# jeremy-rifkin/Markov-Huffman-Coding

Hardware: AMD Instinct MI355X
Metric: encode+decode GB/s on 16 GB byte stream, bit-exact round-trip (higher is better)
Workload: dtype u8

## Files before the change

markov-huffman-coding_amd/csrc/mh_api.cpp:

```cpp
#include "mh_api_internal.hpp"

namespace mhapi {

thread_local int g_last_hip = 0;
thread_local int g_encode_retries = 0;
std::atomic<uint64_t> g_encode_retries_total{0};
thread_local int g_last_index_path = 0;

class PinnedRing {
public:
    static constexpr size_t PIECE = size_t(16) << 20;
    static constexpr int SLOTS = 4;
    hipError_t upload(void *d_dst, const void *h_src, size_t n, hipStream_t st) {
        std::lock_guard<std::mutex> lock(mu_);
        hipError_t e = ensure();
        if (e != hipSuccess) return e;
        const unsigned char *src = static_cast<const unsigned char *>(h_src);
        unsigned char *dst = static_cast<unsigned char *>(d_dst);
        for (size_t off = 0; off < n; off += PIECE, ++seq_) {
            const size_t len = std::min(PIECE, n - off);
            const int s = int(seq_ % SLOTS);
            if ((e = hipEventSynchronize(ev_[s])) != hipSuccess) return e;
            parallel_copy(buf_[s], src + off, len);
            if ((e = hipMemcpyAsync(dst + off, buf_[s], len, hipMemcpyHostToDevice, st)) != hipSuccess) return e;
// ... 363 lines not shown
    p.direct = m->dec_direct ? 1u : 0u; p.H = uint32_t(m->dec_h);
    const int path = decode_path_choice();
    const bool tile_ok = d_fine && path != 2 && (m->type == 2 ? (m->o2_dec_ok && shift <= 10) : (m->tile_p && shift <= 12));
    const bool long_codes = m->type != 2 && nbits && n_symbols && double(nbits) > (double(m->tile_p) - 0.5) * double(n_symbols);
    if (tile_ok && (path == 1 || (n_symbols >= (uint64_t(8) << 20) && !long_codes))) {
        mhk::TileParams t{};
        t.payload = d_payload; t.payload_bytes = p.payload_bytes; t.nbits = nbits; t.d_nbits = p.d_nbits;
        t.out = d_out; t.n = n_symbols; t.index = p.index; t.nchunks = p.nchunks; t.chunk_shift = p.chunk_shift;
        t.fine = d_fine;
        t.prim = m->d_tprim; t.sec = m->d_tsec; t.P = uint32_t(m->tile_p); t.H = uint32_t(m->tile_h); t.nsec = m->tile_nsec;
        if (m->type == 2) {
            t.o2 = 1; t.nslots = m->o2_nslots; t.ctx2slot = m->d_ctx2slot;
            t.prim = reinterpret_cast<const uint16_t *>(m->d_tprim2); t.sec = reinterpret_cast<const uint16_t *>(m->d_tsec2);
            t.P = m->o2_p; t.H = m->o2_h; t.nsec = m->o2_nsec;
        }
        HIP_TRY(mhk::launch_decode_tile(t, p, d_ws, static_cast<hipStream_t>(stream)));
        HIP_TRY(mhk::launch_set_word(reinterpret_cast<uint32_t *>(static_cast<unsigned char *>(d_ws) + 40), mhk::DEC_PATH_TILE, static_cast<hipStream_t>(stream)));
        return MH_OK;
    }
    HIP_TRY(mhk::launch_decode(p, d_ws, static_cast<hipStream_t>(stream)));
    HIP_TRY(mhk::launch_set_word(reinterpret_cast<uint32_t *>(static_cast<unsigned char *>(d_ws) + 40), mhk::DEC_PATH_CHUNK, static_cast<hipStream_t>(stream)));
    return MH_OK;
}

int mh_dev_decode_fine(const mh_model *m, const uint8_t *d_payload, uint64_t nbits, const uint64_t *d_nbits, uint8_t *d_out,
                       uint64_t n_symbols, const uint64_t *d_index, uint32_t chunk_symbols, const uint32_t *d_fine,
                       void *d_ws, size_t ws_bytes, void *stream) {
    return dev_decode(m, d_payload, nbits, d_nbits, d_out, n_symbols, d_index, chunk_symbols, d_ws, ws_bytes, stream, d_fine);
}

int mh_dev_decode(const mh_model *m, const uint8_t *d_payload, uint64_t nbits, uint8_t *d_out, uint64_t n_symbols,
                  const uint64_t *d_index, uint32_t chunk_symbols, void *d_ws, size_t ws_bytes, void *stream) {
    return dev_decode(m, d_payload, nbits, nullptr, d_out, n_symbols, d_index, chunk_symbols, d_ws, ws_bytes, stream);
}

int mh_dev_decode_dn(const mh_model *m, const uint8_t *d_payload, const uint64_t *d_nbits, uint64_t nbits_hint, uint8_t *d_out,
// ... 118 lines not shown
```

markov-huffman-coding_amd/csrc/mh_api_model.cpp:

```cpp
#include "mh_api_internal.hpp"
#include "mh_limit.hpp"

namespace mhapi {

int upload_model(mh_model *m) {
    m->packed = m->host.pack();
    m->type = m->host.type;
    m->max_len = m->packed.max_len;
    m->dec_bits = m->packed.dec_bits; m->dec_h = m->packed.dec_h;
    m->dec_lds = m->packed.dec_lds; m->dec_direct = m->packed.dec_direct;
    m->nsec = uint32_t(m->packed.dec_sec.size());
    for (size_t i = 0; i < size_t(256) * 256; ++i) {
        const int l = m->packed.len8[i];
        if (l && (m->min_len == 0 || l < m->min_len)) m->min_len = l;
    }
    for (int c = 0; c < 256; ++c) {
        int live = 0;
        for (int sy = 0; sy < 256; ++sy) live += m->packed.len8[size_t(c) * 256 + sy] != 0;
        if (live < 2) continue;
        for (int sy = 0; sy < 256; ++sy) m->len_gcd = gcd_u32(m->len_gcd, m->packed.len8[size_t(c) * 256 + sy]);
    }
    if (!have_device()) return MH_OK;
    if (m->max_len > mh::MAX_CODE_BITS) return MH_OK;
    HIP_TRY(hipGetDevice(&m->device));
// ... 200 lines not shown
    for (int i = 0; i < 256; ++i) {
        const int c = order_idx[i];
        const uint32_t *mt = &meta[size_t(c) * mhk::TB_META_STRIDE];
        pa.sec_base_val[c] = uint32_t(nsec);
        nsec += m->dec_direct ? (size_t(mt[3]) << m->dec_h) : size_t(mt[4 + P]);
    }
    m->nsec = uint32_t(nsec);
    const size_t sec_bytes = ((nsec * 2 + 15) & ~size_t(15)) + 16;
    if (d_ws) {
        if (ws_bytes < L.fixed + sec_bytes) return fail(MH_ERR_CAPACITY);
        m->d_sec = reinterpret_cast<uint16_t *>(b + L.fixed);
    } else {
        HIP_TRY_M(hipMalloc(&m->d_sec_own, sec_bytes));
        m->d_sec = static_cast<uint16_t *>(m->d_sec_own);
    }
    HIP_TRY_M(hipMemsetAsync(m->d_sec, 0, sec_bytes, st));
    pa.node_left = m->d_node_left; pa.node_right = m->d_node_right; pa.node_sym = m->d_node_sym; pa.node_height = d_node_height;
    pa.ctx_meta = m->d_meta; pa.sec_base = m->d_sec_base;
    pa.P = uint32_t(P); pa.direct = m->dec_direct ? 1u : 0u; pa.H = uint32_t(m->dec_h); pa.hcap = 8u;
    pa.prim = m->d_prim; pa.sec = m->d_sec; pa.tree = m->d_tree;
    bool packed = false;
    if (const int tP = tile_p_choice()) {
        const int tH = std::min(std::max(m->max_len - tP, 1), 8);
        size_t ntab = size_t(256) << tP;
        mhk::TreePackArgs pt{};
        if (tP == 8) {
            ntab = 0;
            for (int c = 0; c < 256; ++c) { pt.sec_base_val[c] = uint32_t(ntab << tH); ntab += meta[size_t(c) * mhk::TB_META_STRIDE + 3]; }
        } else {
            for (int c = 0; c < 256; ++c) pt.sec_base_val[c] = uint32_t(size_t(c) << (tP + tH));
        }
        if (ntab <= 32767 || tP < 8) {
            const size_t pb = ((size_t(256) << tP) * 2 + 255) & ~size_t(255), sb = (ntab << tH) * 2 + 64;
            unsigned char *tb;
            if (d_ws) {
                const size_t at = (L.fixed + sec_bytes + 255) & ~size_t(255);
                if (ws_bytes < at + pb + sb) return fail(MH_ERR_CAPACITY);
                tb = b + at;
            } else {
                HIP_TRY_M(hipMalloc(&m->d_tile_own, pb + sb));
                tb = static_cast<unsigned char *>(m->d_tile_own);
            }
            m->d_tprim = reinterpret_cast<uint16_t *>(tb);
            m->d_tsec = reinterpret_cast<uint16_t *>(tb + pb);
            HIP_TRY_M(hipMemsetAsync(m->d_tsec, 0, sb, st));
            pt.node_left = m->d_node_left; pt.node_right = m->d_node_right; pt.node_sym = m->d_node_sym; pt.node_height = d_node_height;
            pt.ctx_meta = m->d_meta; pt.sec_base = nullptr; pt.sec_base_in = nullptr;
            pt.P = uint32_t(tP); pt.direct = 1u; pt.H = uint32_t(tH); pt.hcap = 8u;
            pt.prim = m->d_tprim; pt.sec = m->d_tsec; pt.tree = nullptr; pt.lsb = 1u;
            HIP_TRY_M(mhk::launch_tree_pack2(pa, pt, 256, st));
            packed = true;
            m->tile_p = tP; m->tile_h = tH; m->tile_nsec = uint32_t(ntab << tH);
        }
    }
    if (!packed) HIP_TRY_M(mhk::launch_tree_pack(pa, 256, st));
#undef HIP_TRY_M
    *out = m;
    return MH_OK;
}
}

namespace {
constexpr uint32_t O2_CTX = 65536;
constexpr uint32_t O2_HCAP = 4;
const unsigned char O2_MAGIC[4] = {'M', 'H', '2', 1};

bool is_o2_table(const uint8_t *b, size_t n) {
    if (n < 37 || b[0] != 0x80) return false;
    for (int i = 1; i < 33; ++i) if (b[i]) return false;
// ... 505 lines not shown
```

markov-huffman-coding_amd/csrc/mh_decode.hip:

```cpp
#include "mh_decode_dev.hpp"

namespace mhk {

template <typename LS>
__device__ __forceinline__ bool walk_long(const DecTables &t, LS &ls, uint32_t prev, uint32_t e2, uint32_t skip,
                                          uint32_t &sym) {
    ls.buf <<= skip; ls.cnt -= skip;
    uint32_t node = e2 & 0x1FFu;
    const uint32_t *tr = t.tree + prev * TREE_STRIDE;
    for (int guard = 0; guard < 256; ++guard) {
        ls.template refill<true>();
        uint32_t bit = uint32_t(ls.buf >> 63);
        ls.buf <<= 1; ls.cnt -= 1u;
        uint32_t pair = tr[node];
        uint32_t c = bit ? (pair >> 16) : (pair & 0xFFFFu);
        if (c & TREE_LEAF) { sym = c & 255u; ls.template refill<true>(); return true; }
        node = c;
    }
    sym = 0;
    return false;
}

#ifndef MH_DEC_LAG
#define MH_DEC_LAG 1
// ... 128 lines not shown
    }
    for (uint32_t i = nsym & ~3u; i < nsym; ++i) o[i] = uint8_t(q >> (8u * (i & 3u)));
    if (bad || ls[0].position() != uint32_t(end_bits)) atomicExch(status, MHK_STATUS_CORRUPT);
}

template <int K, int OUTB, int NT>
__device__ __forceinline__ void store_burst(const DecParams &p, uint64_t c0, const uint32_t (&Q)[K][OUTB][4], uint32_t b) {
#pragma unroll
    for (int k = 0; k < K; ++k) {
        uint4 *o16 = reinterpret_cast<uint4 *>(p.out + ((c0 + uint64_t(k) * NT) << p.chunk_shift)) + b * OUTB;
#pragma unroll
        for (int u = 0; u < OUTB; ++u) o16[u] = make_uint4(Q[k][u][0], Q[k][u][1], Q[k][u][2], Q[k][u][3]);
    }
}

struct DecCfg { bool sec_lds; int spr; int k, gw, outb, pc, hc; bool redo; int depth; };
__host__ __device__ constexpr DecCfg dec_cfg(int v) {
    return v == DV_LDS_WIDE       ? DecCfg{true, 4, 2, 16, 4, 8, 0, false, 2}
         : v == DV_LDS_SHORT      ? DecCfg{true, 4, 4, 8, 2, 8, 0, false, 2}
         : v == DV_LDS_TWO_LEVEL  ? DecCfg{true, 2, 4, 8, 2, 0, 0, false, 2}
         : v == DV_LDS_TWO_LEVEL_P8 ? DecCfg{true, 2, 4, 8, 2, 8, 0, false, 2}
         : v == DV_L2_DIRECT      ? DecCfg{false, 2, 4, 8, 4, 8, 0, false, 1}
         : v == DV_L2_DIRECT_H2   ? DecCfg{false, 2, 4, 8, 4, 8, 2, false, 1}
         : v == DV_L2_DIRECT_H3   ? DecCfg{false, 2, 4, 8, 4, 8, 3, false, 1}
         : v == DV_L2_DIRECT_H4   ? DecCfg{false, 2, 4, 8, 4, 8, 4, false, 1}
         : v == DV_L2_DIRECT_H8   ? DecCfg{false, 2, 4, 8, 4, 8, 8, false, 1}
         : v == DV_REDO_LDS       ? DecCfg{true, 2, 1, 8, 1, 0, 0, true, 2}
                                  : DecCfg{false, 2, 1, 8, 1, 0, 0, true, 2};
}
constexpr int DEC_NT = 512;
template <int V>
__global__ __launch_bounds__(DEC_NT) void decode_kernel(DecParams p) {
    constexpr DecCfg C = dec_cfg(V);
    constexpr bool SEC_LDS = C.sec_lds, DIRECT = !C.sec_lds, REDO = C.redo;
    constexpr int SPR = C.spr, K = C.k, GW = C.gw, OUTB = C.outb, PC = C.pc, HC = C.hc, NT = DEC_NT, DEPTH = C.depth;
    extern __shared__ __attribute__((aligned(16))) unsigned char smem[];
    if (REDO && p.redo[0] == 0) return;
    if (p.d_nbits) {
        p.nbits = *p.d_nbits;
        p.payload_bytes = (p.nbits + 7) >> 3;
    }
    uint32_t *sub_base = reinterpret_cast<uint32_t *>(smem);
    uint16_t *lut = reinterpret_cast<uint16_t *>(smem + 1024);
    const uint32_t nprim16 = (256u << p.P) / 8u;
    for (uint32_t i = threadIdx.x; i < nprim16; i += NT)
        reinterpret_cast<uint4 *>(lut)[i] = reinterpret_cast<const uint4 *>(p.prim)[i];
    uint16_t *lsec = lut + (256u << p.P);
    if (SEC_LDS) {
        const uint32_t nsec16 = (p.nsec + 7u) / 8u;
        for (uint32_t i = threadIdx.x; i < nsec16; i += NT)
            reinterpret_cast<uint4 *>(lsec)[i] = reinterpret_cast<const uint4 *>(p.sec)[i];
// ... 93 lines not shown
        } else {
            for (int k = 0; k < K; ++k) {
                const uint64_t c = c0 + uint64_t(k) * NT;
                if (c >= p.nchunks) break;
                const uint64_t first = c << p.chunk_shift;
                const uint32_t nsym = (p.n - first) >= S ? S : uint32_t(p.n - first);
                const uint64_t endb = (c + 1 < p.nchunks) ? (p.index[c + 1] & 0x00FFFFFFFFFFFFFFull) : p.nbits;
                decode_chunk_single<DIRECT>(lut, sub_base, tabs, p.payload, p.payload_bytes, p.nbits, p.index[c], endb, p.out + first, nsym, p.status);
            }
        }
    }
}


__global__ __launch_bounds__(256) void decode2_kernel(DecParams p) {
    if (p.d_nbits) { p.nbits = *p.d_nbits; p.payload_bytes = (p.nbits + 7) >> 3; }
    const BitSrc src{p.payload, p.payload_bytes >> 2, p.payload_bytes};
    const DecTables tabs{p.sec, p.tree, p.P, 0u, 0u};
    const uint32_t S = 1u << p.chunk_shift;
    const uint64_t nwork = p.redo_list ? uint64_t(p.redo[0]) : p.nchunks;
    for (uint64_t w = uint64_t(blockIdx.x) * blockDim.x + threadIdx.x; w < nwork; w += uint64_t(gridDim.x) * blockDim.x) {
        const uint64_t c = p.redo_list ? uint64_t(p.redo[1u + w]) : w;
        const uint64_t entry = p.index[c];
        uint64_t pos = entry & IDX2_POS;
        uint32_t ctx = uint32_t(entry >> 48);
        const uint64_t endpos = (c + 1 < p.nchunks) ? (p.index[c + 1] & IDX2_POS) : p.nbits;
        const uint64_t first = c << p.chunk_shift;
        const uint32_t nsym = (p.n - first) >= S ? S : uint32_t(p.n - first);
        if (pos >= p.nbits || endpos < pos || endpos > p.nbits) { atomicExch(p.status, MHK_STATUS_CORRUPT); continue; }
        GranuleCursor bc;
// ... 26 lines not shown
            for (int u = 0; u < 4; ++u) o16[u] = Q[u];
        }
        for (; i < nsym && !bad; ++i) {
            uint32_t used = 0;
            const uint32_t sym = decode_one(p.prim, p.sec_base, tabs, src, bc, ctx, used, bad);
            pos += used;
            ctx = ((ctx << 8) | sym) & 0xFFFFu;
            o[i] = uint8_t(sym);
        }
        if (bad || pos != endpos) atomicExch(p.status, MHK_STATUS_CORRUPT);
    }
}


hipError_t launch_decode_redo(DecParams p, hipStream_t st) {
    if (p.order == 2) {
        p.redo_list = 1;
        const uint64_t want2 = (p.nchunks + 255) / 256;
        const uint64_t cap2 = uint64_t(cu_count()) * 8;
        hipLaunchKernelGGL(decode2_kernel, dim3(unsigned(want2 > cap2 ? cap2 : (want2 < 1 ? 1 : want2))), dim3(256), 0, st, p);
        return hipGetLastError();
    }
    auto r_lds = decode_kernel<DV_REDO_LDS>;
    auto r_l2d = decode_kernel<DV_REDO_L2_DIRECT>;
    hipError_t e = once_per_device(&DeviceState::redo_ready, [&] {
        const void *all[] = {(const void *)r_lds, (const void *)r_l2d};
        for (const void *f : all) {
            hipError_t r = allow_lds(f, DEC_LDS_MAX);
            if (r != hipSuccess) return r;
        }
// ... 2 lines not shown
    if (e != hipSuccess) return e;
    if (!p.sec_lds && !p.direct) return hipErrorInvalidValue;
    if (!p.sec_lds && p.P != 8) return hipErrorInvalidValue;
    const size_t lds = 1024 + (size_t(256) << p.P) * 2 + (p.sec_lds ? ((size_t(p.nsec) * 2 + 15) & ~size_t(15)) : 0);
    if (lds > size_t(DEC_LDS_MAX)) return hipErrorInvalidValue;
    const uint64_t rwant = (p.nchunks + DEC_THREADS - 1) / DEC_THREADS;
    const int rgrid = int(rwant > uint64_t(cu_count()) ? uint64_t(cu_count()) : rwant);
    hipLaunchKernelGGL(p.sec_lds ? r_lds : r_l2d, dim3(rgrid < 1 ? 1 : rgrid), dim3(DEC_THREADS), lds, st, p);
    return hipGetLastError();
}

hipError_t launch_decode(DecParams p, void *d_ws, hipStream_t st) {
    p.status = reinterpret_cast<int *>(d_ws);
    p.redo = reinterpret_cast<uint32_t *>(static_cast<char *>(d_ws) + 64);
    hipError_t e = hipMemsetAsync(d_ws, 0, 64 + 16, st);
    if (e != hipSuccess || p.nchunks == 0) return e;
    if (p.order == 2) {
        const uint64_t want2 = (p.nchunks + 255) / 256;
        const uint64_t cap2 = uint64_t(cu_count()) * 8;
        hipLaunchKernelGGL(decode2_kernel, dim3(unsigned(want2 > cap2 ? cap2 : want2)), dim3(256), 0, st, p);
        return hipGetLastError();
    }
    if (!p.sec_lds && (p.P != 8 || !p.direct)) return hipErrorInvalidValue;
    size_t lds = 1024 + (size_t(256) << p.P) * 2 + (p.sec_lds ? ((size_t(p.nsec) * 2 + 15) & ~size_t(15)) : 0);
    if (lds > size_t(DEC_LDS_MAX)) return hipErrorInvalidValue;
    const bool short_codes = p.nsec == 0 && p.P == 8;
    const bool wide = p.sec_lds && short_codes && p.n > 0 && p.nbits * 10 > p.n * 8 * 6;
    int v;
    if (wide) v = DV_LDS_WIDE;
    else if (p.sec_lds) v = short_codes ? DV_LDS_SHORT : p.P == 8 ? DV_LDS_TWO_LEVEL_P8 : DV_LDS_TWO_LEVEL;
    else v = p.H == 2 ? DV_L2_DIRECT_H2 : p.H == 3 ? DV_L2_DIRECT_H3 : p.H == 4 ? DV_L2_DIRECT_H4 : p.H == 8 ? DV_L2_DIRECT_H8 : DV_L2_DIRECT;
    void (*const kern[DV_REDO_LDS])(DecParams) = {decode_kernel<DV_LDS_WIDE>, decode_kernel<DV_LDS_SHORT>, decode_kernel<DV_LDS_TWO_LEVEL>,
                                                  decode_kernel<DV_LDS_TWO_LEVEL_P8>, decode_kernel<DV_L2_DIRECT>, decode_kernel<DV_L2_DIRECT_H2>,
                                                  decode_kernel<DV_L2_DIRECT_H3>, decode_kernel<DV_L2_DIRECT_H4>, decode_kernel<DV_L2_DIRECT_H8>};
    static_assert(DV_LDS_WIDE == 0 && DV_L2_DIRECT_H8 == 8 && DV_REDO_LDS == 9, "the table above is indexed by DecVariant");
    e = once_per_device(&DeviceState::decode_ready, [&] {
        for (int i = 0; i < DV_REDO_LDS; ++i) {
            hipError_t r = allow_lds(reinterpret_cast<const void *>(kern[i]), DEC_LDS_MAX);
            if (r != hipSuccess) return r;
        }
        return hipSuccess;
    });
    if (e != hipSuccess) return e;
    const uint64_t per_block = uint64_t(DEC_NT) * uint64_t(dec_cfg(v).k);
    const uint64_t want = (p.nchunks + per_block - 1) / per_block;
    const int grid = int(want > uint64_t(cu_count()) ? uint64_t(cu_count()) : want);
    (void)launch_set_word(reinterpret_cast<uint32_t *>(static_cast<char *>(d_ws) + 44), uint32_t(v) + 1u, st);
    hipLaunchKernelGGL(kern[v], dim3(grid), dim3(DEC_NT), lds, st, p);
    e = hipGetLastError();
    if (e != hipSuccess) return e;
    return launch_decode_redo(p, st);
}


}
```

markov-huffman-coding_amd/csrc/mh_encode.hip:

```cpp
#include "mh_dev.hpp"

namespace mhk {


constexpr uint32_t O2H_MAP_OFF = 256, O2H_HOT_OFF = 256 + 64 * 64 * 2;
__device__ __forceinline__ void o2hot_lookup16(const unsigned char *img, const uint4 &x4, uint32_t ctx, uint32_t (&e)[16]) {
    const uint16_t *ctxmap = reinterpret_cast<const uint16_t *>(img + O2H_MAP_OFF);
    const uint16_t *hot = reinterpret_cast<const uint16_t *>(img + O2H_HOT_OFF);
    const uint32_t x[4] = {x4.x, x4.y, x4.z, x4.w};
    uint32_t id[18];
    id[0] = img[ctx >> 8];
    id[1] = img[ctx & 255u];
#pragma unroll
    for (int j = 0; j < 16; ++j) id[2 + j] = img[(x[j >> 2] >> (8 * (j & 3))) & 255u];
    uint32_t cs[16];
#pragma unroll
    for (int j = 0; j < 16; ++j) cs[j] = ctxmap[(id[j] << 6) | (id[j + 1] ^ id[j])];
#pragma unroll
    for (int j = 0; j < 16; ++j) e[j] = hot[(cs[j] << 6) | (id[j + 2] ^ id[j + 1])];
}

__device__ __forceinline__ void o2hot_lookup8(const unsigned char *img, uint32_t xa, uint32_t xb, uint32_t ctx, uint32_t (&e)[8]) {
    const uint16_t *ctxmap = reinterpret_cast<const uint16_t *>(img + O2H_MAP_OFF);
    const uint16_t *hot = reinterpret_cast<const uint16_t *>(img + O2H_HOT_OFF);
// ... 629 lines not shown
            } else if (cur != 0 && lane == 0) {
                stage[0] = 0;
            }
        }
    }
}

constexpr int R_IMG_WORDS = ((163840 - 131072 - 128) / 4) & ~7;
constexpr int R_HALF_WORDS = R_IMG_WORDS / 2;
constexpr uint32_t R_HALF_CAP_BITS = uint32_t(R_HALF_WORDS - 8) * 32u;
static_assert(R_IMG_WORDS >= E_WAVES * (E_STAGE_BITS / 32) + 16 && R_HALF_WORDS % 4 == 0, "image size");
constexpr int REGION_LDS_BYTES = 131072 + R_IMG_WORDS * 4 + 128;



__global__ __launch_bounds__(1024) void region_bits_kernel(const HistHeader *hdr, HistHeader expect, const uint32_t *slab,
                                                           const uint32_t *cross_all, const uint8_t *len8,
                                                           unsigned long long *region_bits, uint32_t *region_esc, int *status) {
    __shared__ unsigned long long part[16];
    __shared__ uint32_t any_esc;
    extern __shared__ __attribute__((aligned(16))) unsigned char lens[];
    for (uint32_t i = threadIdx.x; i < 65536u / 16u; i += 1024u) reinterpret_cast<uint4 *>(lens)[i] = reinterpret_cast<const uint4 *>(len8)[i];
    if (threadIdx.x == 0) any_esc = 0;
    __syncthreads();
    const uint32_t w = blockIdx.x, tid = threadIdx.x;
    if (hdr->magic != HIST_WS_MAGIC || hdr->n != expect.n || hdr->data != expect.data || hdr->region_vecs != expect.region_vecs ||
        hdr->grid != expect.grid || hdr->prev0 != expect.prev0 || hdr->cross_cap != expect.cross_cap) {
        if (tid == 0) { atomicExch(status, MHK_STATUS_CORRUPT); region_bits[w] = 0; region_esc[w] = 0; }
        return;
    }
    unsigned long long acc = 0;
    bool esc = false;
    const uint32_t *sl = slab + size_t(w) * 32768u;
    for (uint32_t i = tid; i < 32768u; i += 1024u) {
        const uint32_t v = sl[i];
        const uint32_t s0 = i, s1 = i | 0x8000u;
        const uint32_t l0 = lens[hist_slot_prev(s0) * 256u + (s0 >> 8)], l1 = lens[hist_slot_prev(s1) * 256u + (s1 >> 8)];
        acc += (unsigned long long)(v & 0xFFFFu) * l0;
        acc += (unsigned long long)(v >> 16) * l1;
        esc |= ((v & 0xFFFFu) && l0 > uint32_t(mh::ENC16_MAX_LEN)) || ((v >> 16) && l1 > uint32_t(mh::ENC16_MAX_LEN));
    }
    const uint32_t *cross = cross_all + size_t(w) * (expect.cross_cap + 1u);
    const uint32_t nc = cross[0];
    if (nc > expect.cross_cap && tid == 0) atomicExch(status, MHK_STATUS_CAPACITY);
    for (uint32_t i = tid; i < (nc < expect.cross_cap ? nc : expect.cross_cap); i += 1024u) {
        const uint32_t sl2 = cross[1u + i];
        const uint32_t l2 = lens[hist_slot_prev(sl2) * 256u + (sl2 >> 8)];
        acc += 16384ull * l2;
        esc |= l2 > uint32_t(mh::ENC16_MAX_LEN);
    }
    if (esc) atomicOr(&any_esc, 1u);
    for (int d = 32; d >= 1; d >>= 1) acc += __shfl_xor(acc, d);
    if ((tid & 63u) == 0) part[tid >> 6] = acc;
    __syncthreads();
    if (tid == 0) {
        unsigned long long t = 0;
        for (int i = 0; i < 16; ++i) t += part[i];
        region_bits[w] = t;
        region_esc[w] = any_esc;
    }
}

__global__ __launch_bounds__(SCAN_THREADS) void region_scan_kernel(const unsigned long long *region_bits, uint32_t nregion,
                                                                   unsigned long long *region_start, const unsigned long long *carry0,
                                                                   uint8_t *out, uint64_t cap, unsigned long long *nbits, int *status) {
    __shared__ uint64_t lds[SCAN_THREADS / 64];
    const uint64_t c0 = carry0 ? (*carry0 & 7ull) : 0;
    const uint32_t i = threadIdx.x;
    const uint64_t v = i < nregion ? region_bits[i] : 0;
    uint64_t total;
    const uint64_t ex = block_excl_scan(v, lds, total);
    const uint64_t s = c0 + ex;
    if (i < nregion) {
        region_start[i] = s;
        if (i > 0 && (s & 31u) && ((s >> 5) + 1) * 4 <= cap) reinterpret_cast<uint32_t *>(out)[s >> 5] = 0;
    }
    if (i == 0) {
        const uint64_t end = c0 + total;
        *nbits = end;
        if (end > cap * 8) atomicExch(status, MHK_STATUS_CAPACITY);
        const uint64_t endw = end >> 5;
        if ((end & 31u) && (endw + 1) * 4 <= cap) reinterpret_cast<uint32_t *>(out)[endw] = 0;
        else if (end & 31u) for (uint64_t b = endw * 4; b < cap; ++b) out[b] = 0;
        if ((c0 & 31u) && 4 <= cap) reinterpret_cast<uint32_t *>(out)[0] = 0;
    }
}

struct RegionParams {
    const unsigned long long *region_start;
    const unsigned long long *region_bits;
    const uint32_t *region_esc;
    uint64_t region_vecs;
    uint64_t nvec_up;
    uint64_t cap_words;
    int *status;
};
constexpr uint32_t R_IMG_CAP_BITS = E_WAVES * E_STAGE_BITS;

struct Roll1 {
// ... 538 lines not shown

hipError_t launch_encode_regions(const EncodeArgs &a, const void *d_hist_ws, size_t hist_ws_bytes, void *d_ws, hipStream_t st) {
    unsigned char *ws = static_cast<unsigned char *>(d_ws);
    int *status = reinterpret_cast<int *>(ws);
    hipError_t e = hipMemsetAsync(ws, 0, 64, st);
    if (e != hipSuccess) return e;
    if (a.n == 0) {
        hipLaunchKernelGGL(empty_payload_kernel, dim3(1), dim3(1), 0, st, a.start_bit, a.nbits, a.out, a.cap);
        return hipGetLastError();
    }
    const RegionGeom g = region_geom(a.n);
    if (!d_hist_ws || hist_ws_bytes < g.total || g.grid > 1024) return hipErrorInvalidValue;
    e = once_per_device(&DeviceState::region_ready, [] {
        hipError_t r = allow_lds(reinterpret_cast<const void *>(enc_region_kernel<false>), REGION_LDS_BYTES);
        if (r == hipSuccess) r = allow_lds(reinterpret_cast<const void *>(enc_region_kernel<false, true>), REGION_LDS_BYTES);
        if (r == hipSuccess) r = allow_lds(reinterpret_cast<const void *>(region_bits_kernel), 65536);
        return r != hipSuccess ? r : allow_lds(reinterpret_cast<const void *>(enc_region_kernel<true>), REGION_LDS_BYTES);
    });
    if (e != hipSuccess) return e;
    const unsigned char *hws = static_cast<const unsigned char *>(d_hist_ws);
    unsigned long long *region_bits = reinterpret_cast<unsigned long long *>(ws + 64);
    unsigned long long *region_start = region_bits + 1024;
    uint32_t *region_esc = reinterpret_cast<uint32_t *>(region_start + 1024);
    const HistHeader expect{HIST_WS_MAGIC, a.n, reinterpret_cast<unsigned long long>(a.data), g.region_vecs, uint32_t(g.grid), a.prev0, g.cross_cap, 0};
    hipLaunchKernelGGL(region_bits_kernel, dim3(g.grid), dim3(1024), 65536, st, reinterpret_cast<const HistHeader *>(hws + 64), expect,
                       reinterpret_cast<const uint32_t *>(hws + g.off_slab), reinterpret_cast<const uint32_t *>(hws + g.off_cross), a.len8,
                       region_bits, region_esc, status);
    hipLaunchKernelGGL(region_scan_kernel, dim3(1), dim3(SCAN_THREADS), 0, st, region_bits, uint32_t(g.grid), region_start, a.start_bit,
                       a.out, a.cap & ~uint64_t(3), a.nbits, status);
    EmitParams ep{a.data, a.n, a.prev0, a.chunk_shift, a.out, a.enc16, a.len8, a.code64, nullptr, nullptr, 0, a.index, status, a.fine, nullptr, 0};
    RegionParams rp{region_start, region_bits, region_esc, g.region_vecs, g.nvec_up, (a.cap & ~uint64_t(3)) >> 2, status};
    (void)launch_set_word(reinterpret_cast<uint32_t *>(ws + 8), uint32_t(a.max_len > mh::ENC16_MAX_LEN ? ENC_PATH_REGIONS_ESCAPES : ENC_PATH_REGIONS), st);
    hipLaunchKernelGGL(enc_region_kernel<false>, dim3(g.grid), dim3(E_THREADS), REGION_LDS_BYTES, st, ep, rp);
    if (a.max_len >= 8)
        hipLaunchKernelGGL((enc_region_kernel<false, true>), dim3(g.grid), dim3(E_THREADS), REGION_LDS_BYTES, st, ep, rp);
    if (a.max_len > mh::ENC16_MAX_LEN)
        hipLaunchKernelGGL(enc_region_kernel<true>, dim3(g.grid), dim3(E_THREADS), REGION_LDS_BYTES, st, ep, rp);
    return hipGetLastError();
}

__global__ __launch_bounds__(256) void enc64_pack_kernel(const uint8_t *len8, const unsigned long long *code64, unsigned long long *enc64, uint64_t n) {
    for (uint64_t i = uint64_t(blockIdx.x) * 256 + threadIdx.x; i < n; i += uint64_t(gridDim.x) * 256) {
        const uint32_t l = len8[i];
        enc64[i] = l <= 56u ? ((unsigned long long)(l) << 56) | code64[i] : 0xFF00000000000000ull;
    }
}
hipError_t launch_enc64_pack(const uint8_t *len8, const uint64_t *code64, uint64_t *enc64, uint64_t n, hipStream_t st) {
// ... 18 lines not shown
```

markov-huffman-coding_amd/csrc/mh_hist.hip:

```cpp
#include "mh_dev.hpp"

namespace mhk {

__global__ void set_word_kernel(uint32_t *p, uint32_t v) { *p = v; }
__global__ void hist_header_kernel(HistHeader *hdr, HistHeader v) { *hdr = v; }
hipError_t launch_set_word(uint32_t *d_word, uint32_t v, hipStream_t st) {
    hipLaunchKernelGGL(set_word_kernel, dim3(1), dim3(1), 0, st, d_word, v);
    return hipGetLastError();
}




template <int GUARD>
__global__ __launch_bounds__(HIST_THREADS) void hist_o1_kernel(const uint8_t *__restrict__ data, uint64_t n,
                                                              uint32_t prev0, unsigned long long *counts, uint32_t *slab,
                                                              uint64_t region_vecs, uint32_t *cross_all, uint32_t cross_cap) {
    constexpr uint32_t CROSS = ((0x10000u - (1u << GUARD)) & 0xFFFFu) * 0x10001u;
    extern __shared__ __attribute__((aligned(16))) unsigned char smem[];
    uint32_t *h = reinterpret_cast<uint32_t *>(smem);
    for (int i = threadIdx.x; i < 32768 / 4; i += HIST_THREADS) reinterpret_cast<uint4 *>(h)[i] = make_uint4(0, 0, 0, 0);
    uint32_t *cross = cross_all ? cross_all + size_t(blockIdx.x) * (cross_cap + 1u) : nullptr;
    if (cross && threadIdx.x == 0) cross[0] = 0;
    __syncthreads();
// ... 64 lines not shown
        uint4 *dst = reinterpret_cast<uint4 *>(slab + size_t(blockIdx.x) * 32768u);
        for (uint32_t i = threadIdx.x; i < 32768u / 4u; i += HIST_THREADS) dst[i] = reinterpret_cast<const uint4 *>(h)[i];
        return;
    }
    for (uint32_t w = threadIdx.x; w < 32768u; w += HIST_THREADS) {
        uint32_t v = h[w];
        uint32_t lo = v & 0xFFFFu, hi = v >> 16;
        if (lo) atomicAdd(&counts[hist_slot_prev(w) * 256u + (w >> 8)], (unsigned long long)lo);
        if (hi) {
            const uint32_t s1 = w | 0x8000u;
            atomicAdd(&counts[hist_slot_prev(s1) * 256u + (s1 >> 8)], (unsigned long long)hi);
        }
    }
}

constexpr uint32_t HIST_REDUCE_WORDS = 64, HIST_REDUCE_SLICES = 4;
__global__ __launch_bounds__(256) void hist_reduce_kernel(const uint32_t *__restrict__ slab, uint32_t nslab, unsigned long long *counts,
                                                          unsigned int *check, unsigned long long n) {
    __shared__ unsigned long long plo[HIST_REDUCE_SLICES][HIST_REDUCE_WORDS], phi[HIST_REDUCE_SLICES][HIST_REDUCE_WORDS];
    const uint32_t col = threadIdx.x & (HIST_REDUCE_WORDS - 1u), slice = threadIdx.x / HIST_REDUCE_WORDS;
    const uint32_t w = blockIdx.x * HIST_REDUCE_WORDS + col;
    const uint32_t per = (nslab + HIST_REDUCE_SLICES - 1u) / HIST_REDUCE_SLICES;
    const uint32_t s_begin = slice * per, s_end = s_begin + per < nslab ? s_begin + per : nslab;
    unsigned long long lo = 0, hi = 0;
    for (uint32_t s = s_begin; s < s_end; ++s) {
        const uint32_t v = slab[size_t(s) * 32768u + w];
        lo += v & 0xFFFFu;
        hi += v >> 16;
    }
    plo[slice][col] = lo; phi[slice][col] = hi;
    __syncthreads();
    if (slice != 0) return;
#pragma unroll
// ... 1 lines not shown
    const uint32_t s1 = w | 0x8000u;
    const unsigned long long c0 = counts[hist_slot_prev(w) * 256u + (w >> 8)] + lo;
    const unsigned long long c1 = counts[hist_slot_prev(s1) * 256u + (s1 >> 8)] + hi;
    counts[hist_slot_prev(w) * 256u + (w >> 8)] = c0;
    counts[hist_slot_prev(s1) * 256u + (s1 >> 8)] = c1;
    if (!check) return;
    unsigned long long t = c0 + c1;
    for (int d = 32; d >= 1; d >>= 1) t += __shfl_xor(t, d);
    if (threadIdx.x == 0) {
        unsigned long long *total = reinterpret_cast<unsigned long long *>(check + 2);
        atomicAdd(total, t);
        __threadfence();
        if (atomicAdd(check + 4, 1u) == gridDim.x - 1u) {
            const unsigned long long all = atomicAdd(total, 0ull);
            if (all != n) atomicExch(reinterpret_cast<int *>(check), MHK_STATUS_CORRUPT);
        }
    }
}

__global__ __launch_bounds__(HIST_THREADS) void hist_o0_kernel(const uint8_t *__restrict__ data, uint64_t n,
                                                              unsigned long long *counts) {
    __shared__ uint32_t h[16][256];
    for (int i = threadIdx.x; i < 16 * 256; i += HIST_THREADS) (&h[0][0])[i] = 0;
    __syncthreads();
    uint32_t *mine = h[threadIdx.x >> 6];
    const uint64_t nvec = n >> 4;
    const uint4 *vdata = reinterpret_cast<const uint4 *>(data);
    for (uint64_t v = uint64_t(blockIdx.x) * HIST_THREADS + threadIdx.x; v < nvec; v += uint64_t(gridDim.x) * HIST_THREADS) {
        uint4 x = vdata[v];
        uint32_t w[4] = {x.x, x.y, x.z, x.w};
// ... 8 lines not shown
    if (blockIdx.x == 0 && threadIdx.x == 0)
        for (uint64_t i = nvec << 4; i < n; ++i) atomicAdd(&mine[data[i]], 1u);
    __syncthreads();
    if (threadIdx.x < 256) {
        unsigned long long s = 0;
        for (int w = 0; w < 16; ++w) s += h[w][threadIdx.x];
        if (s) atomicAdd(&counts[threadIdx.x], s);
    }
}


size_t hist_workspace_bytes(uint64_t n) { return region_geom(n).total; }

hipError_t launch_hist_o1(const uint8_t *d_data, uint64_t n, uint32_t prev0, unsigned long long *d_counts, void *d_ws, size_t ws_bytes,
                          hipStream_t st) {
    hipError_t e = hipMemsetAsync(d_counts, 0, 65536 * sizeof(unsigned long long), st);
    if (e != hipSuccess) return e;
    unsigned char *ws = static_cast<unsigned char *>(d_ws);
    const bool ws_ok = d_ws && (reinterpret_cast<uintptr_t>(d_ws) & 15u) == 0;
    const RegionGeom g = region_geom(n);
    const bool regions = ws_ok && ws_bytes >= g.total;
#ifdef MH_EXP_PROBES
    const char *dbg = getenv("MH_DEBUG_HIST_GUARD_BITS");
    const int guard_bits = dbg ? atoi(dbg) : 2;
#else
    const int guard_bits = 2;
#endif
    const bool guard1 = guard_bits == 0 || guard_bits == 1;
    if (ws_ok && ws_bytes >= 256) {
        e = hipMemsetAsync(ws, 0, 128, st);
        if (e != hipSuccess) return e;
    }
    unsigned int *check = (ws_ok && ws_bytes >= 256) ? reinterpret_cast<unsigned int *>(ws) : nullptr;
    if (regions && !guard1) {
        HistHeader h{HIST_WS_MAGIC, n, reinterpret_cast<unsigned long long>(d_data), g.region_vecs, uint32_t(g.grid), prev0, g.cross_cap, 0};
        hipLaunchKernelGGL(hist_header_kernel, dim3(1), dim3(1), 0, st, reinterpret_cast<HistHeader *>(ws + 64), h);
    }
    if (n == 0) {
        if (regions) { e = hipMemsetAsync(ws + g.off_cross, 0, size_t(g.grid) * (g.cross_cap + 1u) * 4u, st); if (e != hipSuccess) return e;
                       e = hipMemsetAsync(ws + g.off_slab, 0, size_t(g.grid) * 32768u * 4u, st); }
        return e;
    }
    e = once_per_device(&DeviceState::hist_ready, [] {
        hipError_t r = allow_lds(reinterpret_cast<const void *>(hist_o1_kernel<14>), HIST_LDS_BYTES);
#ifdef MH_EXP_PROBES
        if (r == hipSuccess) r = allow_lds(reinterpret_cast<const void *>(hist_o1_kernel<15>), HIST_LDS_BYTES);
        if (r == hipSuccess) r = allow_lds(reinterpret_cast<const void *>(hist_o1_kernel<16>), HIST_LDS_BYTES);
#endif
        return r;
    });
    if (e != hipSuccess) return e;
#ifdef MH_EXP_PROBES
    auto kern = guard_bits == 0 ? hist_o1_kernel<16> : guard_bits == 1 ? hist_o1_kernel<15> : hist_o1_kernel<14>;
#else
    auto kern = hist_o1_kernel<14>;
#endif
    if (regions) {
        uint32_t *slab = reinterpret_cast<uint32_t *>(ws + g.off_slab);
        hipLaunchKernelGGL(kern, dim3(g.grid), dim3(HIST_THREADS), HIST_LDS_BYTES, st, d_data, n, prev0, d_counts, slab,
                           g.region_vecs, reinterpret_cast<uint32_t *>(ws + g.off_cross), g.cross_cap);
        hipLaunchKernelGGL(hist_reduce_kernel, dim3(32768 / HIST_REDUCE_WORDS), dim3(256), 0, st, slab, uint32_t(g.grid), d_counts, check,
                           (unsigned long long)(n));
        return hipGetLastError();
    }
    uint64_t nvec = n >> 4;
    uint64_t want = (nvec + HIST_THREADS - 1) / HIST_THREADS;
    int grid = int(want < 1 ? 1 : (want > uint64_t(cu_count()) ? uint64_t(cu_count()) : want));
    uint32_t *slab = (ws_ok && ws_bytes >= 256 + size_t(grid) * 32768u * 4u) ? reinterpret_cast<uint32_t *>(ws + 256) : nullptr;
    hipLaunchKernelGGL(kern, dim3(grid), dim3(HIST_THREADS), HIST_LDS_BYTES, st, d_data, n, prev0, d_counts, slab,
                       uint64_t(0), static_cast<uint32_t *>(nullptr), 0u);
    if (slab) hipLaunchKernelGGL(hist_reduce_kernel, dim3(32768 / HIST_REDUCE_WORDS), dim3(256), 0, st, slab, uint32_t(grid), d_counts, check,
                                 (unsigned long long)(n));
    return hipGetLastError();
}

hipError_t launch_hist_o0(const uint8_t *d_data, uint64_t n, unsigned long long *d_counts, hipStream_t st) {
    hipError_t e = hipMemsetAsync(d_counts, 0, 256 * sizeof(unsigned long long), st);
    if (e != hipSuccess || n == 0) return e;
    uint64_t nvec = n >> 4;
    uint64_t want = (nvec + HIST_THREADS - 1) / HIST_THREADS;
    int grid = int(want < 1 ? 1 : (want > uint64_t(2 * cu_count()) ? uint64_t(2 * cu_count()) : want));
    hipLaunchKernelGGL(hist_o0_kernel, dim3(grid), dim3(HIST_THREADS), 0, st, d_data, n, d_counts);
    return hipGetLastError();
}


}
// ... 1 lines not shown
```

markov-huffman-coding_amd/csrc/mh_kernels.h:

```cpp
#pragma once

#include <hip/hip_runtime.h>
#include <stddef.h>
#include <stdint.h>

namespace mhk {

enum { MHK_STATUS_OK = 0, MHK_STATUS_TIMEOUT = 1, MHK_STATUS_CAPACITY = 2, MHK_STATUS_CORRUPT = 3 };

struct EncodeArgs {
    int order;
    const uint8_t *data;
    uint64_t n;
    uint32_t prev0;
    uint32_t chunk_shift;
    uint8_t *out;
    uint64_t cap;
    const uint16_t *enc16;
    const uint8_t *len_slot;
    const uint8_t *len8;
    const uint64_t *code64;
    const uint64_t *enc64;
    unsigned long long *nbits;
    unsigned long long *index;
// ... 56 lines not shown
    const unsigned long long *index;
    uint64_t nchunks;
    uint32_t chunk_shift;
    const uint16_t *prim;
    const uint16_t *sec;
    const uint32_t *sec_base;
    const uint32_t *tree;
    uint32_t P;
    uint32_t nsec;
    uint32_t sec_lds;
    uint32_t direct;
    uint32_t H;
    int *status;
    uint32_t *redo;
    uint32_t redo_list;
};

#ifndef MH_T_SUB_SHIFT
#define MH_T_SUB_SHIFT 6
#endif
constexpr int T_SUB_SHIFT = MH_T_SUB_SHIFT;
constexpr uint32_t FINE_POS_MASK = 0x00FFFFFFu;
struct TileParams {
    const uint8_t *payload;
    uint64_t payload_bytes;
    uint64_t nbits;
    const unsigned long long *d_nbits;
    uint8_t *out;
    uint64_t n;
    const unsigned long long *index;
// ... 131 lines not shown
```

Measured before the change: 564.6.

## Fold status-word writes and memsets into kernels to cut tiny launches

Removes several one-thread set_word launches and memsets by writing the decode path/variant words inside the decode kernels, the encode path word inside region_scan_kernel, and the histogram header inside the reduce kernel's last block. Histogram clears become one small kernel, and the model-table memsets are merged into a single contiguous memset where possible. The hist reduce block is widened to 16 slices, and region_bits_kernel transposes the length table in LDS with a padded row to avoid bank conflicts. These cut per-call launch overhead at the cost of more LDS and extra per-kernel conditional writes.

```diff
diff --git a/markov-huffman-coding_amd/csrc/mh_api.cpp b/markov-huffman-coding_amd/csrc/mh_api.cpp
--- a/markov-huffman-coding_amd/csrc/mh_api.cpp
+++ b/markov-huffman-coding_amd/csrc/mh_api.cpp
@@ -401,12 +401,12 @@
             t.prim = reinterpret_cast<const uint16_t *>(m->d_tprim2); t.sec = reinterpret_cast<const uint16_t *>(m->d_tsec2);
             t.P = m->o2_p; t.H = m->o2_h; t.nsec = m->o2_nsec;
         }
+        p.path_word = mhk::DEC_PATH_TILE;
         HIP_TRY(mhk::launch_decode_tile(t, p, d_ws, static_cast<hipStream_t>(stream)));
-        HIP_TRY(mhk::launch_set_word(reinterpret_cast<uint32_t *>(static_cast<unsigned char *>(d_ws) + 40), mhk::DEC_PATH_TILE, static_cast<hipStream_t>(stream)));
         return MH_OK;
     }
+    p.path_word = mhk::DEC_PATH_CHUNK;
     HIP_TRY(mhk::launch_decode(p, d_ws, static_cast<hipStream_t>(stream)));
-    HIP_TRY(mhk::launch_set_word(reinterpret_cast<uint32_t *>(static_cast<unsigned char *>(d_ws) + 40), mhk::DEC_PATH_CHUNK, static_cast<hipStream_t>(stream)));
     return MH_OK;
 }
 
diff --git a/markov-huffman-coding_amd/csrc/mh_api_model.cpp b/markov-huffman-coding_amd/csrc/mh_api_model.cpp
--- a/markov-huffman-coding_amd/csrc/mh_api_model.cpp
+++ b/markov-huffman-coding_amd/csrc/mh_api_model.cpp
@@ -238,7 +238,7 @@
         HIP_TRY_M(hipMalloc(&m->d_sec_own, sec_bytes));
         m->d_sec = static_cast<uint16_t *>(m->d_sec_own);
     }
-    HIP_TRY_M(hipMemsetAsync(m->d_sec, 0, sec_bytes, st));
+    bool sec_cleared = false;
     pa.node_left = m->d_node_left; pa.node_right = m->d_node_right; pa.node_sym = m->d_node_sym; pa.node_height = d_node_height;
     pa.ctx_meta = m->d_meta; pa.sec_base = m->d_sec_base;
     pa.P = uint32_t(P); pa.direct = m->dec_direct ? 1u : 0u; pa.H = uint32_t(m->dec_h); pa.hcap = 8u;
@@ -261,13 +261,19 @@
                 const size_t at = (L.fixed + sec_bytes + 255) & ~size_t(255);
                 if (ws_bytes < at + pb + sb) return fail(MH_ERR_CAPACITY);
                 tb = b + at;
+                HIP_TRY_M(hipMemsetAsync(m->d_sec, 0, at + pb + sb - L.fixed, st));
+                sec_cleared = true;
             } else {
                 HIP_TRY_M(hipMalloc(&m->d_tile_own, pb + sb));
                 tb = static_cast<unsigned char *>(m->d_tile_own);
             }
             m->d_tprim = reinterpret_cast<uint16_t *>(tb);
             m->d_tsec = reinterpret_cast<uint16_t *>(tb + pb);
-            HIP_TRY_M(hipMemsetAsync(m->d_tsec, 0, sb, st));
+            if (!sec_cleared) {
+                HIP_TRY_M(hipMemsetAsync(m->d_sec, 0, sec_bytes, st));
+                HIP_TRY_M(hipMemsetAsync(m->d_tsec, 0, sb, st));
+                sec_cleared = true;
+            }
             pt.node_left = m->d_node_left; pt.node_right = m->d_node_right; pt.node_sym = m->d_node_sym; pt.node_height = d_node_height;
             pt.ctx_meta = m->d_meta; pt.sec_base = nullptr; pt.sec_base_in = nullptr;
             pt.P = uint32_t(tP); pt.direct = 1u; pt.H = uint32_t(tH); pt.hcap = 8u;
@@ -277,6 +283,7 @@
             m->tile_p = tP; m->tile_h = tH; m->tile_nsec = uint32_t(ntab << tH);
         }
     }
+    if (!sec_cleared) HIP_TRY_M(hipMemsetAsync(m->d_sec, 0, sec_bytes, st));
     if (!packed) HIP_TRY_M(mhk::launch_tree_pack(pa, 256, st));
 #undef HIP_TRY_M
     *out = m;
diff --git a/markov-huffman-coding_amd/csrc/mh_decode.hip b/markov-huffman-coding_amd/csrc/mh_decode.hip
--- a/markov-huffman-coding_amd/csrc/mh_decode.hip
+++ b/markov-huffman-coding_amd/csrc/mh_decode.hip
@@ -166,6 +166,13 @@
     }
 }
 
+__device__ __forceinline__ void dec_note_words(const DecParams &p) {
+    if (blockIdx.x == 0 && threadIdx.x == 0) {
+        if (p.path_word) reinterpret_cast<uint32_t *>(p.status)[10] = p.path_word;
+        if (p.variant_word) reinterpret_cast<uint32_t *>(p.status)[11] = p.variant_word;
+    }
+}
+
 struct DecCfg { bool sec_lds; int spr; int k, gw, outb, pc, hc; bool redo; int depth; };
 __host__ __device__ constexpr DecCfg dec_cfg(int v) {
     return v == DV_LDS_WIDE       ? DecCfg{true, 4, 2, 16, 4, 8, 0, false, 2}
@@ -187,6 +194,7 @@
     constexpr bool SEC_LDS = C.sec_lds, DIRECT = !C.sec_lds, REDO = C.redo;
     constexpr int SPR = C.spr, K = C.k, GW = C.gw, OUTB = C.outb, PC = C.pc, HC = C.hc, NT = DEC_NT, DEPTH = C.depth;
     extern __shared__ __attribute__((aligned(16))) unsigned char smem[];
+    dec_note_words(p);
     if (REDO && p.redo[0] == 0) return;
     if (p.d_nbits) {
         p.nbits = *p.d_nbits;
@@ -310,6 +318,7 @@
 
 
 __global__ __launch_bounds__(256) void decode2_kernel(DecParams p) {
+    dec_note_words(p);
     if (p.d_nbits) { p.nbits = *p.d_nbits; p.payload_bytes = (p.nbits + 7) >> 3; }
     const BitSrc src{p.payload, p.payload_bytes >> 2, p.payload_bytes};
     const DecTables tabs{p.sec, p.tree, p.P, 0u, 0u};
@@ -366,6 +375,7 @@
 
 
 hipError_t launch_decode_redo(DecParams p, hipStream_t st) {
+    p.variant_word = 0;
     if (p.order == 2) {
         p.redo_list = 1;
         const uint64_t want2 = (p.nchunks + 255) / 256;
@@ -398,7 +408,8 @@
     p.status = reinterpret_cast<int *>(d_ws);
     p.redo = reinterpret_cast<uint32_t *>(static_cast<char *>(d_ws) + 64);
     hipError_t e = hipMemsetAsync(d_ws, 0, 64 + 16, st);
-    if (e != hipSuccess || p.nchunks == 0) return e;
+    if (e != hipSuccess) return e;
+    if (p.nchunks == 0) return p.path_word ? launch_set_word(reinterpret_cast<uint32_t *>(p.status) + 10, p.path_word, st) : hipSuccess;
     if (p.order == 2) {
         const uint64_t want2 = (p.nchunks + 255) / 256;
         const uint64_t cap2 = uint64_t(cu_count()) * 8;
@@ -429,8 +440,10 @@
     const uint64_t per_block = uint64_t(DEC_NT) * uint64_t(dec_cfg(v).k);
     const uint64_t want = (p.nchunks + per_block - 1) / per_block;
     const int grid = int(want > uint64_t(cu_count()) ? uint64_t(cu_count()) : want);
-    (void)launch_set_word(reinterpret_cast<uint32_t *>(static_cast<char *>(d_ws) + 44), uint32_t(v) + 1u, st);
-    hipLaunchKernelGGL(kern[v], dim3(grid), dim3(DEC_NT), lds, st, p);
+    DecParams m = p;
+    m.variant_word = uint32_t(v) + 1u;
+    m.path_word = 0;
+    hipLaunchKernelGGL(kern[v], dim3(grid), dim3(DEC_NT), lds, st, m);
     e = hipGetLastError();
     if (e != hipSuccess) return e;
     return launch_decode_redo(p, st);
diff --git a/markov-huffman-coding_amd/csrc/mh_encode.hip b/markov-huffman-coding_amd/csrc/mh_encode.hip
--- a/markov-huffman-coding_amd/csrc/mh_encode.hip
+++ b/markov-huffman-coding_amd/csrc/mh_encode.hip
@@ -667,13 +667,21 @@
 
 
 
+constexpr uint32_t REGION_LENS_ROW = 257, REGION_BITS_LDS = 256 * REGION_LENS_ROW;
 __global__ __launch_bounds__(1024) void region_bits_kernel(const HistHeader *hdr, HistHeader expect, const uint32_t *slab,
                                                            const uint32_t *cross_all, const uint8_t *len8,
                                                            unsigned long long *region_bits, uint32_t *region_esc, int *status) {
     __shared__ unsigned long long part[16];
     __shared__ uint32_t any_esc;
     extern __shared__ __attribute__((aligned(16))) unsigned char lens[];
-    for (uint32_t i = threadIdx.x; i < 65536u / 16u; i += 1024u) reinterpret_cast<uint4 *>(lens)[i] = reinterpret_cast<const uint4 *>(len8)[i];
+    for (uint32_t i = threadIdx.x; i < 65536u / 16u; i += 1024u) {
+        const uint4 q = reinterpret_cast<const uint4 *>(len8)[i];
+        const uint32_t qw[4] = {q.x, q.y, q.z, q.w};
+        const uint32_t prev = i >> 4, sym0 = (i & 15u) * 16u;
+#pragma unroll
+        for (uint32_t j = 0; j < 16u; ++j) lens[(sym0 + j) * REGION_LENS_ROW + prev] = uint8_t(qw[j >> 2] >> (8u * (j & 3u)));
+    }
+    auto len_of = [&](uint32_t slot) -> uint32_t { return lens[(slot >> 8) * REGION_LENS_ROW + hist_slot_prev(slot)]; };
     if (threadIdx.x == 0) any_esc = 0;
     __syncthreads();
     const uint32_t w = blockIdx.x, tid = threadIdx.x;
@@ -687,8 +695,7 @@
     const uint32_t *sl = slab + size_t(w) * 32768u;
     for (uint32_t i = tid; i < 32768u; i += 1024u) {
         const uint32_t v = sl[i];
-        const uint32_t s0 = i, s1 = i | 0x8000u;
-        const uint32_t l0 = lens[hist_slot_prev(s0) * 256u + (s0 >> 8)], l1 = lens[hist_slot_prev(s1) * 256u + (s1 >> 8)];
+        const uint32_t l0 = len_of(i), l1 = len_of(i | 0x8000u);
         acc += (unsigned long long)(v & 0xFFFFu) * l0;
         acc += (unsigned long long)(v >> 16) * l1;
         esc |= ((v & 0xFFFFu) && l0 > uint32_t(mh::ENC16_MAX_LEN)) || ((v >> 16) && l1 > uint32_t(mh::ENC16_MAX_LEN));
@@ -697,8 +704,7 @@
     const uint32_t nc = cross[0];
     if (nc > expect.cross_cap && tid == 0) atomicExch(status, MHK_STATUS_CAPACITY);
     for (uint32_t i = tid; i < (nc < expect.cross_cap ? nc : expect.cross_cap); i += 1024u) {
-        const uint32_t sl2 = cross[1u + i];
-        const uint32_t l2 = lens[hist_slot_prev(sl2) * 256u + (sl2 >> 8)];
+        const uint32_t l2 = len_of(cross[1u + i]);
         acc += 16384ull * l2;
         esc |= l2 > uint32_t(mh::ENC16_MAX_LEN);
     }
@@ -716,7 +722,8 @@
 
 __global__ __launch_bounds__(SCAN_THREADS) void region_scan_kernel(const unsigned long long *region_bits, uint32_t nregion,
                                                                    unsigned long long *region_start, const unsigned long long *carry0,
-                                                                   uint8_t *out, uint64_t cap, unsigned long long *nbits, int *status) {
+                                                                   uint8_t *out, uint64_t cap, unsigned long long *nbits, int *status,
+                                                                   uint32_t *path_word, uint32_t path) {
     __shared__ uint64_t lds[SCAN_THREADS / 64];
     const uint64_t c0 = carry0 ? (*carry0 & 7ull) : 0;
     const uint32_t i = threadIdx.x;
@@ -736,6 +743,7 @@
         if ((end & 31u) && (endw + 1) * 4 <= cap) reinterpret_cast<uint32_t *>(out)[endw] = 0;
         else if (end & 31u) for (uint64_t b = endw * 4; b < cap; ++b) out[b] = 0;
         if ((c0 & 31u) && 4 <= cap) reinterpret_cast<uint32_t *>(out)[0] = 0;
+        *path_word = path;
     }
 }
 
@@ -1304,7 +1312,7 @@
     e = once_per_device(&DeviceState::region_ready, [] {
         hipError_t r = allow_lds(reinterpret_cast<const void *>(enc_region_kernel<false>), REGION_LDS_BYTES);
         if (r == hipSuccess) r = allow_lds(reinterpret_cast<const void *>(enc_region_kernel<false, true>), REGION_LDS_BYTES);
-        if (r == hipSuccess) r = allow_lds(reinterpret_cast<const void *>(region_bits_kernel), 65536);
+        if (r == hipSuccess) r = allow_lds(reinterpret_cast<const void *>(region_bits_kernel), REGION_BITS_LDS);
         return r != hipSuccess ? r : allow_lds(reinterpret_cast<const void *>(enc_region_kernel<true>), REGION_LDS_BYTES);
     });
     if (e != hipSuccess) return e;
@@ -1313,14 +1321,14 @@
     unsigned long long *region_start = region_bits + 1024;
     uint32_t *region_esc = reinterpret_cast<uint32_t *>(region_start + 1024);
     const HistHeader expect{HIST_WS_MAGIC, a.n, reinterpret_cast<unsigned long long>(a.data), g.region_vecs, uint32_t(g.grid), a.prev0, g.cross_cap, 0};
-    hipLaunchKernelGGL(region_bits_kernel, dim3(g.grid), dim3(1024), 65536, st, reinterpret_cast<const HistHeader *>(hws + 64), expect,
+    hipLaunchKernelGGL(region_bits_kernel, dim3(g.grid), dim3(1024), REGION_BITS_LDS, st, reinterpret_cast<const HistHeader *>(hws + 64), expect,
                        reinterpret_cast<const uint32_t *>(hws + g.off_slab), reinterpret_cast<const uint32_t *>(hws + g.off_cross), a.len8,
                        region_bits, region_esc, status);
     hipLaunchKernelGGL(region_scan_kernel, dim3(1), dim3(SCAN_THREADS), 0, st, region_bits, uint32_t(g.grid), region_start, a.start_bit,
-                       a.out, a.cap & ~uint64_t(3), a.nbits, status);
+                       a.out, a.cap & ~uint64_t(3), a.nbits, status, reinterpret_cast<uint32_t *>(ws + 8),
+                       uint32_t(a.max_len > mh::ENC16_MAX_LEN ? ENC_PATH_REGIONS_ESCAPES : ENC_PATH_REGIONS));
     EmitParams ep{a.data, a.n, a.prev0, a.chunk_shift, a.out, a.enc16, a.len8, a.code64, nullptr, nullptr, 0, a.index, status, a.fine, nullptr, 0};
     RegionParams rp{region_start, region_bits, region_esc, g.region_vecs, g.nvec_up, (a.cap & ~uint64_t(3)) >> 2, status};
-    (void)launch_set_word(reinterpret_cast<uint32_t *>(ws + 8), uint32_t(a.max_len > mh::ENC16_MAX_LEN ? ENC_PATH_REGIONS_ESCAPES : ENC_PATH_REGIONS), st);
     hipLaunchKernelGGL(enc_region_kernel<false>, dim3(g.grid), dim3(E_THREADS), REGION_LDS_BYTES, st, ep, rp);
     if (a.max_len >= 8)
         hipLaunchKernelGGL((enc_region_kernel<false, true>), dim3(g.grid), dim3(E_THREADS), REGION_LDS_BYTES, st, ep, rp);
diff --git a/markov-huffman-coding_amd/csrc/mh_hist.hip b/markov-huffman-coding_amd/csrc/mh_hist.hip
--- a/markov-huffman-coding_amd/csrc/mh_hist.hip
+++ b/markov-huffman-coding_amd/csrc/mh_hist.hip
@@ -4,6 +4,11 @@
 
 __global__ void set_word_kernel(uint32_t *p, uint32_t v) { *p = v; }
 __global__ void hist_header_kernel(HistHeader *hdr, HistHeader v) { *hdr = v; }
+__global__ __launch_bounds__(1024) void hist_clear_kernel(unsigned long long *counts, unsigned long long *ws128) {
+    const uint32_t i = blockIdx.x * 1024u + threadIdx.x;
+    counts[i] = 0;
+    if (ws128 && i < 16u) ws128[i] = 0;
+}
 hipError_t launch_set_word(uint32_t *d_word, uint32_t v, hipStream_t st) {
     hipLaunchKernelGGL(set_word_kernel, dim3(1), dim3(1), 0, st, d_word, v);
     return hipGetLastError();
@@ -102,9 +107,9 @@
     }
 }
 
-constexpr uint32_t HIST_REDUCE_WORDS = 64, HIST_REDUCE_SLICES = 4;
-__global__ __launch_bounds__(256) void hist_reduce_kernel(const uint32_t *__restrict__ slab, uint32_t nslab, unsigned long long *counts,
-                                                          unsigned int *check, unsigned long long n) {
+constexpr uint32_t HIST_REDUCE_WORDS = 64, HIST_REDUCE_SLICES = 16;
+__global__ __launch_bounds__(HIST_REDUCE_WORDS * HIST_REDUCE_SLICES) void hist_reduce_kernel(const uint32_t *__restrict__ slab, uint32_t nslab, unsigned long long *counts,
+                                                          unsigned int *check, unsigned long long n, HistHeader *hdr, HistHeader hdr_val) {
     __shared__ unsigned long long plo[HIST_REDUCE_SLICES][HIST_REDUCE_WORDS], phi[HIST_REDUCE_SLICES][HIST_REDUCE_WORDS];
     const uint32_t col = threadIdx.x & (HIST_REDUCE_WORDS - 1u), slice = threadIdx.x / HIST_REDUCE_WORDS;
     const uint32_t w = blockIdx.x * HIST_REDUCE_WORDS + col;
@@ -136,6 +141,7 @@
         if (atomicAdd(check + 4, 1u) == gridDim.x - 1u) {
             const unsigned long long all = atomicAdd(total, 0ull);
             if (all != n) atomicExch(reinterpret_cast<int *>(check), MHK_STATUS_CORRUPT);
+            if (hdr) *hdr = hdr_val;
         }
     }
 }
@@ -174,8 +180,6 @@
 
 hipError_t launch_hist_o1(const uint8_t *d_data, uint64_t n, uint32_t prev0, unsigned long long *d_counts, void *d_ws, size_t ws_bytes,
                           hipStream_t st) {
-    hipError_t e = hipMemsetAsync(d_counts, 0, 65536 * sizeof(unsigned long long), st);
-    if (e != hipSuccess) return e;
     unsigned char *ws = static_cast<unsigned char *>(d_ws);
     const bool ws_ok = d_ws && (reinterpret_cast<uintptr_t>(d_ws) & 15u) == 0;
     const RegionGeom g = region_geom(n);
@@ -187,15 +191,14 @@
     const int guard_bits = 2;
 #endif
     const bool guard1 = guard_bits == 0 || guard_bits == 1;
-    if (ws_ok && ws_bytes >= 256) {
-        e = hipMemsetAsync(ws, 0, 128, st);
-        if (e != hipSuccess) return e;
-    }
     unsigned int *check = (ws_ok && ws_bytes >= 256) ? reinterpret_cast<unsigned int *>(ws) : nullptr;
-    if (regions && !guard1) {
-        HistHeader h{HIST_WS_MAGIC, n, reinterpret_cast<unsigned long long>(d_data), g.region_vecs, uint32_t(g.grid), prev0, g.cross_cap, 0};
-        hipLaunchKernelGGL(hist_header_kernel, dim3(1), dim3(1), 0, st, reinterpret_cast<HistHeader *>(ws + 64), h);
-    }
+    hipLaunchKernelGGL(hist_clear_kernel, dim3(64), dim3(1024), 0, st, d_counts, reinterpret_cast<unsigned long long *>(check));
+    hipError_t e = hipGetLastError();
+    if (e != hipSuccess) return e;
+    const bool with_hdr = regions && !guard1;
+    const HistHeader h{HIST_WS_MAGIC, n, reinterpret_cast<unsigned long long>(d_data), g.region_vecs, uint32_t(g.grid), prev0, g.cross_cap, 0};
+    HistHeader *d_hdr = with_hdr ? reinterpret_cast<HistHeader *>(ws + 64) : nullptr;
+    if (with_hdr && n == 0) hipLaunchKernelGGL(hist_header_kernel, dim3(1), dim3(1), 0, st, d_hdr, h);
     if (n == 0) {
         if (regions) { e = hipMemsetAsync(ws + g.off_cross, 0, size_t(g.grid) * (g.cross_cap + 1u) * 4u, st); if (e != hipSuccess) return e;
                        e = hipMemsetAsync(ws + g.off_slab, 0, size_t(g.grid) * 32768u * 4u, st); }
@@ -219,8 +222,8 @@
         uint32_t *slab = reinterpret_cast<uint32_t *>(ws + g.off_slab);
         hipLaunchKernelGGL(kern, dim3(g.grid), dim3(HIST_THREADS), HIST_LDS_BYTES, st, d_data, n, prev0, d_counts, slab,
                            g.region_vecs, reinterpret_cast<uint32_t *>(ws + g.off_cross), g.cross_cap);
-        hipLaunchKernelGGL(hist_reduce_kernel, dim3(32768 / HIST_REDUCE_WORDS), dim3(256), 0, st, slab, uint32_t(g.grid), d_counts, check,
-                           (unsigned long long)(n));
+        hipLaunchKernelGGL(hist_reduce_kernel, dim3(32768 / HIST_REDUCE_WORDS), dim3(HIST_REDUCE_WORDS * HIST_REDUCE_SLICES), 0, st, slab, uint32_t(g.grid), d_counts, check,
+                           (unsigned long long)(n), d_hdr, h);
         return hipGetLastError();
     }
     uint64_t nvec = n >> 4;
@@ -229,8 +232,8 @@
     uint32_t *slab = (ws_ok && ws_bytes >= 256 + size_t(grid) * 32768u * 4u) ? reinterpret_cast<uint32_t *>(ws + 256) : nullptr;
     hipLaunchKernelGGL(kern, dim3(grid), dim3(HIST_THREADS), HIST_LDS_BYTES, st, d_data, n, prev0, d_counts, slab,
                        uint64_t(0), static_cast<uint32_t *>(nullptr), 0u);
-    if (slab) hipLaunchKernelGGL(hist_reduce_kernel, dim3(32768 / HIST_REDUCE_WORDS), dim3(256), 0, st, slab, uint32_t(grid), d_counts, check,
-                                 (unsigned long long)(n));
+    if (slab) hipLaunchKernelGGL(hist_reduce_kernel, dim3(32768 / HIST_REDUCE_WORDS), dim3(HIST_REDUCE_WORDS * HIST_REDUCE_SLICES), 0, st, slab, uint32_t(grid), d_counts, check,
+                                 (unsigned long long)(n), static_cast<HistHeader *>(nullptr), h);
     return hipGetLastError();
 }
 
diff --git a/markov-huffman-coding_amd/csrc/mh_kernels.h b/markov-huffman-coding_amd/csrc/mh_kernels.h
--- a/markov-huffman-coding_amd/csrc/mh_kernels.h
+++ b/markov-huffman-coding_amd/csrc/mh_kernels.h
@@ -94,6 +94,8 @@
     int *status;
     uint32_t *redo;
     uint32_t redo_list;
+    uint32_t path_word;
+    uint32_t variant_word;
 };
 
 #ifndef MH_T_SUB_SHIFT
```

Result: no change. 564.2 (-0.1%).
